# UCLALibrary/jp2-bucketeer

Measured on AMD Instinct MI355X. Metric: encoded megapixels/sec (node), lossless 5/3 + lossy 9/7, at 1/2/4/8 MI355X, higher is better.
Workload: dtype f32+i32

## Files before the change

jp2-bucketeer_amd/csrc/t1.hip:

```cpp
#include <hip/hip_runtime.h>

#include <algorithm>
#include <cstdlib>
#include <cstring>

#include "device_common.h"
#include "gpu_encoder.h"

namespace jp2hip {

enum { CX_RL = 17, CX_UNI = 18, CX_PAD = 19 };
constexpr uint8_t kPadDecision = CX_PAD << 1;



constexpr int kCmWaves = 2;

__device__ __forceinline__ int order_bucket(uint32_t n) {
    const uint32_t v = n + 1u;
    const int e = 31 - __clz(v);
    constexpr int kLog = kOrderSub == 16 ? 4 : 3;
    const int f = e >= kLog ? (int)((v >> (e - kLog)) & (kOrderSub - 1u)) : (int)((v << (kLog - e)) & (kOrderSub - 1u));
    return kOrderBuckets - 1 - min(kOrderBuckets - 1, kOrderSub * e + f);
}


constexpr uint64_t kStripeTop = 0x1111111111111111ull;
constexpr uint64_t kStripeBot = 0x8888888888888888ull;

__device__ __forceinline__ uint64_t col_left(uint64_t x, int) { return wave_shr1(x); }
__device__ __forceinline__ uint64_t col_right(uint64_t x, int) { return wave_shl1(x); }

struct Nbr8 {
    uint64_t UL, U, UR, L, R, DL, D, DR;
};
__device__ __forceinline__ Nbr8 nbr8(uint64_t Vb, uint64_t Va, uint64_t LVb, uint64_t RVb, uint64_t LVa,
                                     uint64_t RVa) {
    Nbr8 n;
    n.UL = LVb << 1;
    n.U = Vb << 1;
    n.UR = ((RVb << 1) & kStripeTop) | ((RVa << 1) & ~kStripeTop);
    n.L = LVb;
    n.R = RVa;
    n.DL = ((LVa >> 1) & kStripeBot) | ((LVb >> 1) & ~kStripeBot);
    n.D = Va >> 1;
    n.DR = RVa >> 1;
    return n;
}

template <uint32_t TT>
__device__ __forceinline__ uint64_t b3(uint64_t a, uint64_t b, uint64_t c) {
    const uint32_t lo = __builtin_amdgcn_bitop3_b32((uint32_t)a, (uint32_t)b, (uint32_t)c, TT);
    const uint32_t hi = __builtin_amdgcn_bitop3_b32((uint32_t)(a >> 32), (uint32_t)(b >> 32), (uint32_t)(c >> 32), TT);
    return ((uint64_t)hi << 32) | lo;
}

struct Ctx4 {
    uint64_t b0, b1, b2, b3;
};
__device__ __forceinline__ Ctx4 zc_masks(int band, const Nbr8 &n) {
    const uint64_t u = n.UL | n.UR, d = n.DL | n.DR, dge1 = u | d;
    const uint64_t s2a = n.DL & n.DR;
    const uint64_t dge2 = b3<0xEA>(u, d, b3<0xEA>(n.UL, n.UR, s2a));
    Ctx4 z;
    if (band == 3) {
        const uint64_t dge3 = b3<0xEA>(s2a, u, (n.UL & n.UR) & d);
        const uint64_t a = n.L | n.R, c = n.U | n.D, hvge1 = a | c;
        const uint64_t hvge2 = b3<0xEA>(a, c, b3<0xEA>(n.L, n.R, n.U & n.D));
        const uint64_t d2 = b3<0x30>(dge2, dge3, dge3), d1 = b3<0x30>(dge1, dge2, dge2);
        const uint64_t hv1 = b3<0x30>(hvge1, hvge2, hvge2);
        z.b3 = dge3;
        z.b2 = b3<0xEA>(d1, hvge1, d2);
        z.b1 = b3<0xAE>(dge1, hvge2, b3<0xBA>(d1, hvge1, d2));
        z.b0 = b3<0xEA>(d2, hvge1, b3<0x72>(d1, dge1, hv1));
    } else {
        const uint64_t A1 = band == 1 ? n.U : n.L, A2 = band == 1 ? n.D : n.R;
        const uint64_t B1 = band == 1 ? n.L : n.U, B2 = band == 1 ? n.R : n.D;
        const uint64_t e = b3<0x30>(dge1, dge2, dge2);
        const uint64_t x = A1 ^ A2;
        z.b3 = A1 & A2;
        z.b2 = b3<0x3E>(A1, A2, B1 & B2);
        z.b1 = b3<0xEA>(x, B1 | B2 | dge1, b3<0x02>(A1, A2, b3<0x3E>(B1, B2, dge2)));
        z.b0 = b3<0xEA>(x, b3<0xFD>(B1, B2, dge1), b3<0x02>(A1, A2, b3<0x3E>(B1, B2, e)));
    }
    return z;
}

struct Sc4 {
    uint64_t b0, b1, b2, xr;
};
__device__ __forceinline__ void sc_pair(uint64_t As, uint64_t An, uint64_t Bs, uint64_t Bn, uint64_t &p, uint64_t &n) {
    const uint64_t nA = As & An, nB = Bs & Bn;
    const uint64_t pA = b3<0x30>(As, An, An), pB = b3<0x30>(Bs, Bn, Bn);
    p = b3<0xBA>(pB, nA, b3<0x10>(As, An, nB));
    n = b3<0xBA>(nB, pA, b3<0x30>(nA, pB, pB));
}
__device__ __forceinline__ Sc4 sc_masks(uint64_t Ls, uint64_t Ln, uint64_t Rs, uint64_t Rn, uint64_t Us, uint64_t Un,
                                        uint64_t Ds, uint64_t Dn) {
    uint64_t hp, hn, vp, vn;
    sc_pair(Ls, Ln, Rs, Rn, hp, hn);
    sc_pair(Us, Un, Ds, Dn, vp, vn);
    const uint64_t hnz = hp | hn, vnz = vp | vn;
    const uint64_t opp = b3<0xEA>(hn, vp, hp & vn);
    Sc4 c;
    c.b0 = ~(hnz ^ vnz);
    c.b1 = b3<0xAE>(hnz, vnz, opp);
    c.b2 = b3<0x30>(hnz, opp, opp);
    c.xr = b3<0xF2>(hn, hnz, vn);
    return c;
}


constexpr int kRingBytes = 4096;
constexpr int kRingGuard = 4;
constexpr int kRingWords = kRingBytes / 4 + kRingGuard;
constexpr int kCm3Blocks = 4096;

__device__ __forceinline__ uint32_t spread4(uint32_t nib) { return (nib * 0x00204081u) & 0x01010101u; }
__device__ __forceinline__ uint32_t spread4s(uint32_t nib, int k) {
    return __umul24(nib << k, 0x00204081u) & (0x01010101u << k);
}
__device__ __forceinline__ uint32_t nibw(uint32_t w, int sh) { return __builtin_amdgcn_ubfe(w, (uint32_t)sh, 4u); }

struct Ring {
    uint32_t *r;
    uint8_t *out;
    int pos, fl;
};

template <int NW>
__device__ __forceinline__ void ring_or(const Ring &g, uint32_t at, uint32_t o0, uint32_t o1, uint32_t o2,
                                        uint32_t n) {
    const uint32_t t = at & 3u;
    const uint32_t sel = 0x07060504u - __builtin_amdgcn_perm(0u, t, 0u);
    uint32_t *q = g.r + ((at >> 2) & (uint32_t)(kRingBytes / 4 - 1));
    if (n) {
        atomicOr(q, o0 << (8u * t));
        atomicOr(q + 1, __builtin_amdgcn_perm(o1, o0, sel));
        if (NW >= 3) atomicOr(q + 2, __builtin_amdgcn_perm(o2, o1, sel));
        if (NW >= 4) atomicOr(q + 3, __builtin_amdgcn_perm(0u, o2, sel));
    }
}

template <int NW>
__device__ __forceinline__ void ring_put2(Ring &g, uint32_t a0, uint32_t a1, uint32_t a2, uint32_t na, uint32_t b0,
                                          uint32_t b1, uint32_t b2, uint32_t nb) {
    const uint32_t n = na | (nb << 16);
    int v = (int)n;
    v += __builtin_amdgcn_update_dpp(0, v, 0x111, 0xf, 0xf, false);
    v += __builtin_amdgcn_update_dpp(0, v, 0x112, 0xf, 0xf, false);
    v += __builtin_amdgcn_update_dpp(0, v, 0x114, 0xf, 0xf, false);
    v += __builtin_amdgcn_update_dpp(0, v, 0x118, 0xf, 0xf, false);
    v += __builtin_amdgcn_update_dpp(0, v, 0x142, 0xa, 0xf, false);
    v += __builtin_amdgcn_update_dpp(0, v, 0x143, 0xc, 0xf, false);
    const uint32_t tot = (uint32_t)__builtin_amdgcn_readlane(v, 63);
    const uint32_t ex = (uint32_t)v - n;
    const uint32_t ta = tot & 0xFFFFu;
    ring_or<NW>(g, (uint32_t)g.pos + (ex & 0xFFFFu), a0, a1, a2, na);
    ring_or<NW>(g, (uint32_t)g.pos + ta + (ex >> 16), b0, b1, b2, nb);
    g.pos += (int)(ta + (tot >> 16));
}

__device__ __forceinline__ void ring_drain(Ring &g, int upto, int lane) {
    if (lane < kRingGuard) {
        const uint32_t gv = g.r[kRingBytes / 4 + lane];
        if (gv) {
            g.r[lane] |= gv;
            g.r[kRingBytes / 4 + lane] = 0u;
        }
    }
    __builtin_amdgcn_wave_barrier();
    for (int o = g.fl + 16 * lane; o < upto; o += 1024) {
        uint4 *src = (uint4 *)((uint8_t *)g.r + (o & (kRingBytes - 1)));
        const uint4 v = *src;
        *src = make_uint4(0u, 0u, 0u, 0u);
        *(uint4 *)(g.out + o) = v;
    }
    g.fl = __builtin_amdgcn_readfirstlane(upto);
}

__device__ __forceinline__ void ring_step(Ring &g, int lane) {
    if (__builtin_amdgcn_readfirstlane(g.pos - g.fl) >= 1024) ring_drain(g, g.fl + 1024, lane);
}

__device__ __forceinline__ void ring_pass_end(Ring &g, int lane) {
    const int end = (g.pos + 15) & ~15;
    if (lane < end - g.pos) ((uint8_t *)g.r)[(g.pos + lane) & (kRingBytes - 1)] = kPadDecision;
    ring_drain(g, end, lane);
    g.pos = end;
}

struct Half {
    uint32_t mem, bb, z0, z1, z2, z3, c0, c1, c2, xs, x;
};
__device__ __forceinline__ Half half_of(int hf, uint64_t mem, uint64_t bb, const Ctx4 &z, const Sc4 &sc, uint64_t xs,
                                        uint64_t x) {
    const int sh = hf * 32;
    return Half{(uint32_t)(mem >> sh),  (uint32_t)(bb >> sh),    (uint32_t)(z.b0 >> sh), (uint32_t)(z.b1 >> sh),
                (uint32_t)(z.b2 >> sh), (uint32_t)(z.b3 >> sh),  (uint32_t)(sc.b0 >> sh), (uint32_t)(sc.b1 >> sh),
                (uint32_t)(sc.b2 >> sh), (uint32_t)(xs >> sh), (uint32_t)(x >> sh)};
}
__device__ __forceinline__ uint32_t spread_or(uint32_t w, int sh, int k, uint32_t acc) {
    const uint32_t nib = nibw(w, sh);
    if (k <= 2) return (__umul24(nib, 0x00204081u << k) & (0x01010101u << k)) | acc;
    return spread4s(nib, k) | acc;
}
__device__ __forceinline__ void zc_sg_bytes(const Half &m, int sh, uint32_t &zc, uint32_t &sg) {
    zc = spread_or(m.bb, sh, 0, 0u);
    zc = spread_or(m.z0, sh, 1, zc);
    zc = spread_or(m.z1, sh, 2, zc);
    zc = spread_or(m.z2, sh, 3, zc);
    zc = spread_or(m.z3, sh, 4, zc);
    sg = spread_or(m.xs, sh, 0, 0x10101010u);
    sg = spread_or(m.c0, sh, 1, sg);
    sg = spread_or(m.c1, sh, 2, sg);
    sg = spread_or(m.c2, sh, 3, sg);
}

__device__ __forceinline__ void spp_stripe(const Half &m, int sh, const uint2 *lut, uint32_t &o0, uint32_t &o1,
                                           uint32_t &n) {
    const uint32_t mem = nibw(m.mem, sh);
    uint32_t zc, sg;
    zc_sg_bytes(m, sh, zc, sg);
    const uint32_t K = mem | ((mem & nibw(m.bb, sh)) << 4);
    const uint2 sel = lut[K];
    o0 = __builtin_amdgcn_perm(sg, zc, sel.x);
    o1 = __builtin_amdgcn_perm(sg, zc, sel.y);
    n = (uint32_t)__popc(K);
}
__device__ __forceinline__ void mrp_stripe(uint32_t wm, uint32_t wb, uint32_t wf, uint32_t wa, int sh,
                                           const uint2 *lut, uint32_t &o0, uint32_t &n) {
    const uint32_t mem = nibw(wm, sh);
    const uint32_t f = spread4(nibw(wf, sh));
    const uint32_t mr = (0x20202020u - (f << 2)) | spread_or(wa, sh, 1, spread4(nibw(wb, sh)));
    o0 = __builtin_amdgcn_perm(0u, mr, lut[mem].x);
    n = (uint32_t)__popc(mem);
}
__device__ __forceinline__ void cup_stripe(const Half &m, int sh, const uint2 *lut, uint32_t &o0, uint32_t &o1,
                                           uint32_t &o2, uint32_t &n) {
    const uint32_t mem = nibw(m.mem, sh);
    uint32_t zc, sg;
    zc_sg_bytes(m, sh, zc, sg);
    const uint32_t bb = nibw(m.bb, sh);
    const bool rl = mem == 0xFu && nibw(m.x, sh) == 0u;
    const uint32_t r = __builtin_ctz(bb | 16u);
    const uint32_t mr = rl ? (0xEu << r) & 0xFu : mem;
    const uint32_t K = mr | ((mr & bb) << 4);
    const uint2 sel = lut[K];
    o0 = __builtin_amdgcn_perm(sg, zc, sel.x);
    o1 = __builtin_amdgcn_perm(sg, zc, sel.y);
    o2 = 0u;
    n = (uint32_t)__popc(K);
    if (rl) {
        if (bb == 0u) {
            o0 = (uint32_t)(CX_RL << 1);
            n = 1;
        } else {
            o2 = o1;
            o1 = o0;
            o0 = (uint32_t)((CX_RL << 1) | 1) | ((uint32_t)((CX_UNI << 1) | (r >> 1)) << 8) |
                 ((uint32_t)((CX_UNI << 1) | (r & 1u)) << 16) | (((sg >> (8 * r)) & 0xFFu) << 24);
            n += 4;
        }
    }
}

__device__ __forceinline__ uint32_t cm_plane(const T1CmArgs &a, Ring &g, const uint2 *lut, int lane, int b, int k,
                                             int p, int P, int w, int h, int band, const uint64_t *CT, uint64_t B,
                                             uint64_t S0, uint64_t S1, uint64_t S2, uint64_t SG, uint64_t LSG,
                                             uint64_t RSG) {
    const bool lossless = a.lossless != 0;
    const bool vl = lane < w;
    const uint64_t VR = vl ? (h >= 64 ? ~0ull : ((1ull << h) - 1ull)) : 0ull;
    const int nstripes = (h + 3) >> 2;
    g.out = a.stream + a.slot_off[b] + (size_t)k * plane_stream_cap(w, h);
    g.pos = 0;
    g.fl = 0;
    int n_spp = 0, n_mrp = 0;
    const bool spp = p < P - 1;
    const uint64_t LS1 = col_left(S1, lane), RS1 = col_right(S1, lane);
    uint64_t N = 0, memS = 0;
    if (spp) {
        for (;;) {
            const uint64_t Vb = S1 | N, LVb = col_left(Vb, lane), RVb = col_right(Vb, lane);
            const Nbr8 nb = nbr8(Vb, S1, LVb, RVb, LS1, RS1);
            const uint64_t cand = ~S1 & VR & (nb.UL | nb.U | nb.UR | nb.L | nb.R | nb.DL | nb.D | nb.DR);
            const uint64_t Nn = cand & B;
            if (!__any(Nn != N)) {
                memS = cand;
                break;
            }
            N = Nn;
        }
        {
            const uint64_t Vb = S1 | N, LVb = col_left(Vb, lane), RVb = col_right(Vb, lane);
            const Nbr8 nb = nbr8(Vb, S1, LVb, RVb, LS1, RS1);
            const Ctx4 z = zc_masks(band, nb);
            const Sc4 sc = sc_masks(nb.L, LSG, nb.R, RSG, nb.U, SG << 1, nb.D, SG >> 1);
            for (int hf = 0; hf * 8 < nstripes; hf++) {
                const Half m = half_of(hf, memS, B, z, sc, SG ^ sc.xr, 0);
                for (int s4 = 0; s4 < 8 && hf * 8 + s4 < nstripes; s4 += 2) {
                    const int sh = s4 * 4;
                    const bool hb = hf * 8 + s4 + 1 < nstripes;
                    if (!__any(nibw(m.mem, sh) | (hb ? nibw(m.mem, sh + 4) : 0u))) continue;
                    uint32_t a0, a1, ca, b0 = 0, b1 = 0, cb = 0;
                    spp_stripe(m, sh, lut, a0, a1, ca);
                    if (hb) spp_stripe(m, sh + 4, lut, b0, b1, cb);
                    ring_put2<3>(g, a0, a1, 0u, ca, b0, b1, 0u, cb);
                    ring_step(g, lane);
                }
            }
        }
        n_spp = g.pos;
        ring_pass_end(g, lane);
        const int mrp0 = g.pos;
        {
            const uint64_t Pst = S1 | N, LP = col_left(Pst, lane), RP = col_right(Pst, lane);
            const uint64_t anyn = (Pst << 1) | (Pst >> 1) | LP | RP | (LP << 1) | (RP << 1) | (LP >> 1) | (RP >> 1);
            const uint64_t memM = S1 & VR, fr = S1 & ~S2, fa = fr & anyn;
            for (int hf = 0; hf * 8 < nstripes; hf++) {
                const int hs = hf * 32;
                const uint32_t wm = (uint32_t)(memM >> hs), wb = (uint32_t)(B >> hs), wf = (uint32_t)(fr >> hs),
                               wa = (uint32_t)(fa >> hs);
                for (int s4 = 0; s4 < 8 && hf * 8 + s4 < nstripes; s4 += 2) {
                    const int sh = s4 * 4;
                    const bool hb = hf * 8 + s4 + 1 < nstripes;
                    if (!__any(nibw(wm, sh) | (hb ? nibw(wm, sh + 4) : 0u))) continue;
                    uint32_t a0, ca, b0 = 0, cb = 0;
                    mrp_stripe(wm, wb, wf, wa, sh, lut, a0, ca);
                    if (hb) mrp_stripe(wm, wb, wf, wa, sh + 4, lut, b0, cb);
                    ring_put2<2>(g, a0, 0u, 0u, ca, b0, 0u, 0u, cb);
                    ring_step(g, lane);
                }
            }
        }
        n_mrp = g.pos - mrp0;
        ring_pass_end(g, lane);
    }
    const int cup0 = g.pos;
    {
        const uint64_t Pst = S1 | N, LP = col_left(Pst, lane), RP = col_right(Pst, lane);
        const uint64_t LS0 = col_left(S0, lane), RS0 = col_right(S0, lane);
        const Nbr8 nb = nbr8(S0, Pst, LS0, RS0, LP, RP);
        const Ctx4 z = zc_masks(band, nb);
        const Sc4 sc = sc_masks(nb.L, LSG, nb.R, RSG, nb.U, SG << 1, nb.D, SG >> 1);
        const uint64_t memC = ~S1 & ~memS & VR;
        const uint64_t side = LS0 | RP, above = S0 | LS0 | RS0, below = Pst | LP | RP;
        const uint64_t blk = side | ((above << 1) & kStripeTop) | ((below >> 1) & kStripeBot);
        for (int hf = 0; hf * 8 < nstripes; hf++) {
            const Half m = half_of(hf, memC, B, z, sc, SG ^ sc.xr, blk);
            for (int s4 = 0; s4 < 8 && hf * 8 + s4 < nstripes; s4 += 2) {
                const int sh = s4 * 4;
                const bool hb = hf * 8 + s4 + 1 < nstripes;
                if (!__any(nibw(m.mem, sh) | (hb ? nibw(m.mem, sh + 4) : 0u))) continue;
                uint32_t a0, a1, a2, ca, b0 = 0, b1 = 0, b2 = 0, cb = 0;
                cup_stripe(m, sh, lut, a0, a1, a2, ca);
                if (hb) cup_stripe(m, sh + 4, lut, b0, b1, b2, cb);
                ring_put2<4>(g, a0, a1, a2, ca, b0, b1, b2, cb);
                ring_step(g, lane);
            }
        }
    }
    const int n_cup = g.pos - cup0;
    ring_pass_end(g, lane);
    int64_t dspp = 0;
    if (spp && __any(N != 0ull)) {
        const uint32_t nl = (uint32_t)__popcll(N);
        int64_t sv = (int64_t)nl << p;
#pragma unroll 4
        for (int q = 0; q < p; q++) sv += (int64_t)__popcll(N & CT[(size_t)q * 64 + lane]) << q;
        const int64_t nN = (int64_t)wave_sum_u32(nl);
        sv = wave_sum64(sv);
        dspp = (lossless && p == 0) ? 4 * nN
                                    : ((12 * sv + (6 * (lossless ? 0 : 1) - 9 * ((int64_t)1 << p)) * nN) << p);
    }
    if (lane == 0) {
        uint4 cnt;
        cnt.x = (uint32_t)n_spp;
        cnt.y = (uint32_t)n_mrp;
        cnt.z = (uint32_t)n_cup;
        cnt.w = 0;
        a.counts[(size_t)b * 32 + k] = cnt;
        a.dspp[(size_t)b * 32 + k] = dspp;
    }
    return (uint32_t)(n_spp + n_mrp + n_cup);
}

__device__ __forceinline__ uint2 cm_selectors(int K) {
    uint64_t sel = 0x0C0C0C0C0C0C0C0Cull;
    int n = 0;
#pragma unroll
    for (int q = 0; q < 8; q++) {
        const int bit = (q & 1) ? 4 + (q >> 1) : (q >> 1);
        if ((K >> bit) & 1) {
            sel = (sel & ~(0xFFull << (8 * n))) | ((uint64_t)((q & 1) ? 4 + (q >> 1) : (q >> 1)) << (8 * n));
            n++;
        }
    }
    return make_uint2((uint32_t)sel, (uint32_t)(sel >> 32));
}

struct CmBlk {
    int b, P, c, w, h, Mb, band;
    uint64_t bp_off, slot;
};
__device__ __forceinline__ CmBlk cm_blk_load(const T1CmArgs &a, int b) {
    const BlockDesc d = a.blocks[b];
    CmBlk k;
    k.b = b;
    k.P = a.P[b];
    k.c = (int)(a.acc[b] >> 40);
    k.w = d.w;
    k.h = d.h;
    k.Mb = d.Mb;
    k.band = d.band;
    k.bp_off = d.bp_off;
    k.slot = a.slot_off[b];
    return k;
}
struct CmMasks {
    uint64_t SG, B;
};
__device__ __forceinline__ CmMasks cm_masks_load(const T1CmArgs &a, const CmBlk &k, int lane) {
    const uint64_t *CT = a.bp + k.bp_off;
    CmMasks m;
    m.SG = CT[(size_t)k.Mb * 64 + lane];
    m.B = CT[(size_t)(k.P - 1) * 64 + lane];
    return m;
}

#ifdef JP2HIP_CM_WAVES_PER_EU
__global__ void __launch_bounds__(64 * kCmWaves) __attribute__((amdgpu_waves_per_eu(JP2HIP_CM_WAVES_PER_EU))) k_t1_cm3(T1CmArgs a) {
#else
__global__ void __launch_bounds__(64 * kCmWaves) k_t1_cm3(T1CmArgs a) {
#endif
    __shared__ uint2 lut[256];
    __shared__ uint32_t rings[kCmWaves][kRingWords];
    const int lane = threadIdx.x & 63;
    const int wv = __builtin_amdgcn_readfirstlane(threadIdx.x >> 6);
    for (int K = threadIdx.x; K < 256; K += 64 * kCmWaves) lut[K] = cm_selectors(K);
    for (int i = threadIdx.x; i < kCmWaves * kRingWords; i += 64 * kCmWaves) (&rings[0][0])[i] = 0u;
    __syncthreads();
    const int nblk = a.kmax > 0 ? (int)a.dfill[0] : 0;
    Ring g;
    g.r = rings[wv];
    const int stride = gridDim.x * kCmWaves;
    int bi = blockIdx.x * kCmWaves + wv;
    if (bi >= nblk) return;
    CmBlk cur = cm_blk_load(a, a.dlist[bi]);
    CmMasks mk = cm_masks_load(a, cur, lane);
    int idx_next = bi + stride < nblk ? a.dlist[bi + stride] : -1;
    for (;;) {
        const int b = cur.b, P = cur.P, c = cur.c, w = cur.w, h = cur.h, band = cur.band;
        const bool vl = lane < w;
        const uint64_t *CT = a.bp + cur.bp_off;
        uint64_t Bl = mk.B;
        const uint64_t SG = vl ? mk.SG : 0ull;
        const uint64_t LSG = col_left(SG, lane), RSG = col_right(SG, lane);
        uint64_t S1 = 0, S2 = 0;
        uint32_t tot = 0;
        const uint32_t cap = plane_stream_cap(w, h);
        uint8_t *out = a.stream + cur.slot;
        CmBlk nxt;
        int idx_after = -1;
        for (int k = 0; k < c; k++) {
            const int p = P - 1 - k;
            const uint64_t B = vl ? Bl : 0ull, S0 = S1 | B;
            if (k + 1 < c) Bl = CT[(size_t)(p - 1) * 64 + lane];
            if (k == 0 && idx_next >= 0) {
                nxt = cm_blk_load(a, idx_next);
                if (bi + 2 * stride < nblk) idx_after = a.dlist[bi + 2 * stride];
            }
            g.out = out + (size_t)k * cap;
            g.pos = 0;
            g.fl = 0;
            tot += cm_plane(a, g, lut, lane, b, k, p, P, w, h, band, CT, B, S0, S1, S2, SG, LSG, RSG);
#ifdef JP2HIP_BURN_VALU
            {
                uint32_t x = (uint32_t)B ^ (uint32_t)lane;
                for (int i = 0; i < JP2HIP_BURN_VALU; i++) x = (x ^ (uint32_t)i) + (x << 3);
                if (x == 0x9E3779B9u) a.counts[(size_t)b * 32 + k].w = x;
            }
#endif
#ifdef JP2HIP_BURN_SLEEP
            __builtin_amdgcn_s_sleep(JP2HIP_BURN_SLEEP);
#endif
            S2 = S1;
            S1 = S0;
        }
        const bool more = idx_next >= 0;
        if (more) mk = cm_masks_load(a, nxt, lane);
        if (lane == 0) {
            a.acc[b] = tot;
            const int bk = order_bucket(tot);
            a.bslots[(size_t)bk * a.nb + atomicAdd(&a.bfill[bk], 1u)] = b;
        }
        if (!more) break;
        bi += stride;
        cur = nxt;
        idx_next = idx_after;
    }
}

__constant__ uint16_t c_qe[47] = {
    0x5601, 0x3401, 0x1801, 0x0AC1, 0x0521, 0x0221, 0x5601, 0x5401, 0x4801, 0x3801, 0x3001, 0x2401,
    0x1C01, 0x1601, 0x5601, 0x5401, 0x5101, 0x4801, 0x3801, 0x3401, 0x3001, 0x2801, 0x2401, 0x2201,
    0x1C01, 0x1801, 0x1601, 0x1401, 0x1201, 0x1101, 0x0AC1, 0x09C1, 0x08A1, 0x0521, 0x0441, 0x02A1,
    0x0221, 0x0141, 0x0111, 0x0085, 0x0049, 0x0025, 0x0015, 0x0009, 0x0005, 0x0001, 0x5601};
__constant__ uint8_t c_nmps[47] = {1,  2,  3,  4,  5,  38, 7,  8,  9,  10, 11, 12, 13, 29, 15, 16,
                                   17, 18, 19, 20, 21, 22, 23, 24, 25, 26, 27, 28, 29, 30, 31, 32,
                                   33, 34, 35, 36, 37, 38, 39, 40, 41, 42, 43, 44, 45, 45, 46};
__constant__ uint8_t c_nlps[47] = {1,  6,  9,  12, 29, 33, 6,  14, 14, 14, 17, 18, 20, 21, 14, 14,
                                   15, 16, 17, 18, 19, 19, 20, 21, 22, 23, 24, 25, 26, 27, 28, 29,
                                   30, 31, 32, 33, 34, 35, 36, 37, 38, 39, 40, 41, 42, 43, 46};

struct Mq {
    uint32_t C, A, B;
    int CT, bp, cap;
    uint8_t *out;
};

__device__ __forceinline__ void mq_byteout(Mq &m) {
    uint32_t B = m.B;
    if (B != 0xFF && m.C >= 0x8000000u) {
        B++;
        m.C &= 0x7FFFFFFu;
    }
    if (m.bp >= 0 && m.bp < m.cap) m.out[m.bp] = (uint8_t)B;
    m.bp++;
    if (B == 0xFF) {
        m.B = m.C >> 20;
        m.C &= 0xFFFFFu;
        m.CT = 7;
    } else {
        m.B = m.C >> 19;
        m.C &= 0x7FFFFu;
        m.CT = 8;
    }
}

__device__ __forceinline__ uint32_t ring_at(int bp, uint32_t lb) {
    uint32_t r;
    asm("v_bfi_b32 %0, 63, %1, %2" : "=v"(r) : "v"(bp), "v"(lb));
    return r;
}

__device__ __forceinline__ void ring_byteout(Mq &m, uint8_t *ring, uint32_t lb) {
    uint32_t B = m.B;
    if (B != 0xFF && m.C >= 0x8000000u) {
        B++;
        m.C &= 0x7FFFFFFu;
    }
    ring[ring_at(m.bp, lb)] = (uint8_t)B;
    m.bp++;
    const bool ff = B == 0xFF;
    m.B = ff ? (m.C >> 20) : (m.C >> 19);
    m.C &= ff ? 0xFFFFFu : 0x7FFFFu;
    m.CT = ff ? 7 : 8;
}

constexpr int kMqChunk = 16;
#ifndef JP2HIP_MQ_EXP
#define JP2HIP_MQ_EXP 0
#endif
constexpr uint32_t kPadWord = 0x01010101u * kPadDecision;
constexpr int kQeShift = 16;
#ifndef JP2HIP_MQ_SCHED
#define JP2HIP_MQ_SCHED 1
#endif
#ifndef JP2HIP_MQ_PASS_PREFETCH
#define JP2HIP_MQ_PASS_PREFETCH 1
#endif


__device__ __forceinline__ uint32_t mq_word(int e) {
    return ((uint32_t)c_qe[e >> 1] << kQeShift) | ((uint32_t)e << 3) | (uint32_t)(e & 1);
}

__device__ __forceinline__ uint32_t mq_model(uint32_t &A, const uint32_t t, const uint8_t *tab, const uint32_t d,
                                             uint32_t *code) {
#if JP2HIP_MQ_EXP == 3
    const uint2 nx = make_uint2(t ^ 0x10008u, t ^ 0x20010u);
#else
    const uint2 nx = *(const uint2 *)(tab + (t & 0x3F8u));
#endif
    const uint32_t qe = t & 0xFFFF0000u;
    const bool isM = d == (t & 1u);
    const uint32_t A1 = A - qe;
    const bool keep = isM != (A1 < qe);
    const uint32_t An = keep ? A1 : qe;
    const bool ren = !isM || A1 < 0x80000000u;
    const uint32_t n = (uint32_t)__builtin_clz(An);
    A = An << n;
    const uint32_t cw = (keep ? qe : 0u) | n;
#if JP2HIP_MQ_SCHED
    __builtin_amdgcn_sched_barrier(0);
#endif
    *code = cw;
    return ren ? (isM ? nx.x : nx.y) : t;
}

template <bool TWO>
__device__ __forceinline__ void mq_code(Mq &m, const uint32_t code, uint8_t *ring, uint32_t lb) {
    const uint32_t add = code >> kQeShift;
    const int n = (int)(code & 0x1Fu);
    const uint32_t C0 = m.C + add;
    const int CT = m.CT;
    const bool bo = n >= CT;
    const int s1 = min(n, CT);
    const uint32_t C1 = C0 << s1;
    const bool carry = (m.B != 0xFFu) && (C1 >= 0x8000000u);
    const uint32_t Bc = m.B + (carry ? 1u : 0u);
    const uint32_t C2 = carry ? (C1 & 0x7FFFFFFu) : C1;
    const bool ff = Bc == 0xFFu;
    const uint32_t sh = ff ? 20u : 19u;
    ring[ring_at(m.bp, lb)] = (uint8_t)Bc;
    uint32_t Cx = bo ? (C2 & ((1u << sh) - 1u)) : C1;
    int CTx = bo ? 27 - (int)sh : CT - n;
    int rem = n - s1;
    m.B = bo ? (C2 >> sh) : m.B;
    m.bp += bo ? 1 : 0;
    if (TWO && bo && rem >= CTx) {
        m.C = Cx << CTx;
        rem -= CTx;
        ring_byteout(m, ring, lb);
        Cx = m.C;
        CTx = m.CT;
    }
    m.C = Cx << rem;
    m.CT = CTx - rem;
}

__device__ __forceinline__ void ring_flush(const Mq &m, const uint8_t *ring, uint32_t lb, int off, int &fl) {
    while (m.bp - fl >= 16) {
        uint4 v;
        v.x = *(const uint32_t *)(ring + ring_at(fl, lb));
        v.y = *(const uint32_t *)(ring + ring_at(fl + 4, lb));
        v.z = *(const uint32_t *)(ring + ring_at(fl + 8, lb));
        v.w = *(const uint32_t *)(ring + ring_at(fl + 12, lb));
        if (fl - off + 16 <= m.cap) *(uint4 *)(m.out + (fl - off)) = v;
        fl += 16;
    }
}

__device__ __forceinline__ int mq_flush(Mq &m) {
    uint32_t tempc = m.C + m.A;
    m.C |= 0xFFFFu;
    if (m.C >= tempc) m.C -= 0x8000u;
    m.C <<= m.CT;
    mq_byteout(m);
    m.C <<= m.CT;
    mq_byteout(m);
    if (m.B != 0xFF) {
        if (m.bp >= 0 && m.bp < m.cap) m.out[m.bp] = (uint8_t)m.B;
        m.bp++;
    }
    return m.bp;
}

struct MqShared {
    uint2 mqt[94];
    uint32_t cxs[20 * 64];
    uint32_t rings[64 * 16];
    union {
        uint32_t bbase[kOrderBuckets + 1];
        uint32_t code[2][kMqChunk][64];
    };
    int32_t segs[2][64];
    uint32_t finA[64];
    int32_t blk[64];
    int32_t more[2];
#ifdef JP2HIP_MQ_LDS_PAD
    uint8_t pad_[JP2HIP_MQ_LDS_PAD];
#endif
};

__device__ __forceinline__ void mq_modeller(const T1MqArgs &a, MqShared &sh) {
    const int lane = threadIdx.x & 63;
    const int b = sh.blk[lane];
    uint32_t *cx = sh.cxs + lane;
    const uint8_t *mqt = (const uint8_t *)sh.mqt;
    const uint32_t w0 = mq_word(0);
#pragma unroll
    for (int q = 0; q < 19; q++) cx[q * 64] = w0;
    cx[CX_PAD * 64] = 0u;
    cx[0] = mq_word(2 * 4);
    cx[CX_RL * 64] = mq_word(2 * 3);
    cx[CX_UNI * 64] = mq_word(2 * 46);
    uint32_t A = 0x8000u << kQeShift;
    int nseg = 0, s = 0, k = 0, pass = 2, left = 0, Pt = 0;
    uint32_t cap = 0;
    const uint8_t *sbase = nullptr;
    const uint4 *cntp = nullptr, *ptr = nullptr;
    const int64_t *dspp = nullptr, *dref = nullptr, *dsig = nullptr;
    int64_t *D = nullptr;
    const uint4 pad4 = make_uint4(kPadWord, kPadWord, kPadWord, kPadWord);
    uint4 cnt = make_uint4(0u, 0u, 0u, 0u), cur = pad4, nx1 = pad4;
    int64_t ndec = 0;
#if JP2HIP_MQ_PASS_PREFETCH
    int pf_pass = 0, pf_k = 0, pf_valid = 0;
    uint4 pf_cnt = cnt, pf_cur = pad4, pf_nx1 = pad4;
    const uint4 *pf_ptr = nullptr;
    auto prefetch = [&]() {
        pf_valid = 0;
        if (s + 1 >= nseg) return;
        const int np = pass == 2 ? 0 : pass + 1, nk = pass == 2 ? k + 1 : k;
        const uint4 nc = np == 0 ? cntp[nk] : cnt;
        const int o_mrp = ((int)cnt.x + 15) & ~15;
        const int o_cup = (o_mrp + (int)cnt.y + 15) & ~15;
        pf_ptr = (const uint4 *)(sbase + (size_t)nk * cap + (np == 0 ? 0 : (np == 1 ? o_mrp : o_cup)));
        pf_cur = pf_ptr[0];
        pf_nx1 = pf_ptr[1];
        pf_pass = np;
        pf_k = nk;
        pf_cnt = nc;
        pf_valid = 1;
    };
#endif
    if (b >= 0) {
        const BlockDesc d = a.blocks[b];
        Pt = a.P[b];
        const int P = Pt - a.pmin[b];
        nseg = 3 * P - 2;
        D = a.dists + (size_t)b * kMaxPasses;
        cap = plane_stream_cap(d.w, d.h);
        sbase = a.stream + a.slot_off[b];
        cntp = a.counts + (size_t)b * 32;
        dspp = a.dspp + (size_t)b * 32;
        dref = a.dref + (size_t)b * 32;
        dsig = a.dsig + (size_t)b * 32;
        cnt = cntp[0];
        ptr = (const uint4 *)sbase;
        left = (int)cnt.z;
        ndec = left;
        cur = ptr[0];
        if (left > 16) nx1 = ptr[1];
#if JP2HIP_MQ_PASS_PREFETCH
        prefetch();
#endif
    }
    uint64_t cyc_wait = 0;
    const uint64_t cyc0 = __builtin_readcyclecounter();
    for (int it = 0;; it++) {
        while (left <= 0 && s < nseg) {
#if JP2HIP_MQ_PASS_PREFETCH
            if (++s >= nseg) break;
            pass = pf_pass;
            k = pf_k;
            cnt = pf_cnt;
            ptr = pf_ptr;
            cur = pf_cur;
            nx1 = pf_nx1;
            left = pass == 0 ? (int)cnt.x : (pass == 1 ? (int)cnt.y : (int)cnt.z);
            ndec += left;
            prefetch();
#else
            const int p = Pt - 1 - k;
            D[s] = pass == 0 ? dspp[k] : (pass == 1 ? dref[p] : dsig[p] - dspp[k]);
            if (++s >= nseg) break;
            pass = pass == 2 ? 0 : pass + 1;
            if (pass == 0) {
                k++;
                cnt = cntp[k];
            }
            const int o_mrp = ((int)cnt.x + 15) & ~15;
            const int o_cup = (o_mrp + (int)cnt.y + 15) & ~15;
            ptr = (const uint4 *)(sbase + (size_t)k * cap + (pass == 0 ? 0 : (pass == 1 ? o_mrp : o_cup)));
            left = pass == 0 ? (int)cnt.x : (pass == 1 ? (int)cnt.y : (int)cnt.z);
            ndec += left;
            cur = ptr[0];
            nx1 = left > 16 ? ptr[1] : pad4;
#endif
        }
        const bool active = s < nseg;
        const int buf = it & 1;
        sh.segs[buf][lane] = s;
        if (!__any(active)) {
            sh.finA[lane] = A >> kQeShift;
            if (lane == 0) sh.more[buf] = 0;
// ... 194 lines not shown
```

Measured before the change: 34670.

## Fuse SPP, MRP and cleanup passes into one stripe sweep with per-pass rings

The three coding passes (significance propagation, magnitude refinement, cleanup) per bit-plane used to run as three separate stripe sweeps through one shared LDS ring. Now a single sweep emits all three into separate per-pass LDS rings. The MRP/SPP output offsets are precomputed from wave-wide popcounts, and the cleanup neighbourhood is built by selecting the SPP neighbourhood under the SPP membership mask. This removes two of the three sweeps and the repeated mask and context setup, but it raises register pressure and LDS use and adds extra scans per stripe. The default waves-per-EU attribute is also now always set to 4.

```diff
diff --git a/jp2-bucketeer_amd/csrc/t1.hip b/jp2-bucketeer_amd/csrc/t1.hip
--- a/jp2-bucketeer_amd/csrc/t1.hip
+++ b/jp2-bucketeer_amd/csrc/t1.hip
@@ -111,9 +111,13 @@
 }
 
 
-constexpr int kRingBytes = 4096;
 constexpr int kRingGuard = 4;
-constexpr int kRingWords = kRingBytes / 4 + kRingGuard;
+constexpr int kRingSpp = 2048, kDrainSpp = 1024, kStripeSpp = 512;
+constexpr int kRingMrp = 1024, kDrainMrp = 512, kStripeMrp = 256;
+constexpr int kRingCup = 2048, kDrainCup = 512, kStripeCup = 768;
+constexpr int kRingWordsSpp = kRingSpp / 4 + kRingGuard, kRingWordsMrp = kRingMrp / 4 + kRingGuard,
+              kRingWordsCup = kRingCup / 4 + kRingGuard;
+constexpr int kWaveRingWords = kRingWordsSpp + kRingWordsMrp + kRingWordsCup;
 constexpr int kCm3Blocks = 4096;
 
 __device__ __forceinline__ uint32_t spread4(uint32_t nib) { return (nib * 0x00204081u) & 0x01010101u; }
@@ -122,18 +126,18 @@
 }
 __device__ __forceinline__ uint32_t nibw(uint32_t w, int sh) { return __builtin_amdgcn_ubfe(w, (uint32_t)sh, 4u); }
 
+template <int BYTES>
 struct Ring {
     uint32_t *r;
-    uint8_t *out;
     int pos, fl;
 };
 
-template <int NW>
-__device__ __forceinline__ void ring_or(const Ring &g, uint32_t at, uint32_t o0, uint32_t o1, uint32_t o2,
+template <int NW, int BYTES>
+__device__ __forceinline__ void ring_or(const Ring<BYTES> &g, uint32_t at, uint32_t o0, uint32_t o1, uint32_t o2,
                                         uint32_t n) {
     const uint32_t t = at & 3u;
     const uint32_t sel = 0x07060504u - __builtin_amdgcn_perm(0u, t, 0u);
-    uint32_t *q = g.r + ((at >> 2) & (uint32_t)(kRingBytes / 4 - 1));
+    uint32_t *q = g.r + ((at >> 2) & (uint32_t)(BYTES / 4 - 1));
     if (n) {
         atomicOr(q, o0 << (8u * t));
         atomicOr(q + 1, __builtin_amdgcn_perm(o1, o0, sel));
@@ -142,64 +146,44 @@
     }
 }
 
-template <int NW>
-__device__ __forceinline__ void ring_put2(Ring &g, uint32_t a0, uint32_t a1, uint32_t a2, uint32_t na, uint32_t b0,
-                                          uint32_t b1, uint32_t b2, uint32_t nb) {
-    const uint32_t n = na | (nb << 16);
-    int v = (int)n;
-    v += __builtin_amdgcn_update_dpp(0, v, 0x111, 0xf, 0xf, false);
-    v += __builtin_amdgcn_update_dpp(0, v, 0x112, 0xf, 0xf, false);
-    v += __builtin_amdgcn_update_dpp(0, v, 0x114, 0xf, 0xf, false);
-    v += __builtin_amdgcn_update_dpp(0, v, 0x118, 0xf, 0xf, false);
-    v += __builtin_amdgcn_update_dpp(0, v, 0x142, 0xa, 0xf, false);
-    v += __builtin_amdgcn_update_dpp(0, v, 0x143, 0xc, 0xf, false);
-    const uint32_t tot = (uint32_t)__builtin_amdgcn_readlane(v, 63);
-    const uint32_t ex = (uint32_t)v - n;
-    const uint32_t ta = tot & 0xFFFFu;
-    ring_or<NW>(g, (uint32_t)g.pos + (ex & 0xFFFFu), a0, a1, a2, na);
-    ring_or<NW>(g, (uint32_t)g.pos + ta + (ex >> 16), b0, b1, b2, nb);
-    g.pos += (int)(ta + (tot >> 16));
-}
-
-__device__ __forceinline__ void ring_drain(Ring &g, int upto, int lane) {
+template <int BYTES>
+__device__ __forceinline__ void ring_drain(Ring<BYTES> &g, uint8_t *out, int upto, int lane) {
     if (lane < kRingGuard) {
-        const uint32_t gv = g.r[kRingBytes / 4 + lane];
+        const uint32_t gv = g.r[BYTES / 4 + lane];
         if (gv) {
             g.r[lane] |= gv;
-            g.r[kRingBytes / 4 + lane] = 0u;
+            g.r[BYTES / 4 + lane] = 0u;
         }
     }
     __builtin_amdgcn_wave_barrier();
     for (int o = g.fl + 16 * lane; o < upto; o += 1024) {
-        uint4 *src = (uint4 *)((uint8_t *)g.r + (o & (kRingBytes - 1)));
+        uint4 *src = (uint4 *)((uint8_t *)g.r + (o & (BYTES - 1)));
         const uint4 v = *src;
         *src = make_uint4(0u, 0u, 0u, 0u);
-        *(uint4 *)(g.out + o) = v;
+        *(uint4 *)(out + o) = v;
     }
     g.fl = __builtin_amdgcn_readfirstlane(upto);
 }
 
-__device__ __forceinline__ void ring_step(Ring &g, int lane) {
-    if (__builtin_amdgcn_readfirstlane(g.pos - g.fl) >= 1024) ring_drain(g, g.fl + 1024, lane);
-}
-
-__device__ __forceinline__ void ring_pass_end(Ring &g, int lane) {
+template <int DRAIN, int ADD, int BYTES>
+__device__ __forceinline__ void ring_step(Ring<BYTES> &g, uint8_t *out, int lane) {
+    static_assert(DRAIN % 16 == 0 && DRAIN - 1 + ADD < BYTES, "ring_step: pending bytes must fit the ring");
+    const int pend = __builtin_amdgcn_readfirstlane(g.pos - g.fl);
+    if (pend >= DRAIN) ring_drain(g, out, g.fl + (pend & ~15), lane);
+}
+
+template <int BYTES>
+__device__ __forceinline__ void ring_pass_end(Ring<BYTES> &g, uint8_t *out, int lane) {
     const int end = (g.pos + 15) & ~15;
-    if (lane < end - g.pos) ((uint8_t *)g.r)[(g.pos + lane) & (kRingBytes - 1)] = kPadDecision;
-    ring_drain(g, end, lane);
+    if (end == g.fl) return;
+    if (lane < end - g.pos) ((uint8_t *)g.r)[(g.pos + lane) & (BYTES - 1)] = kPadDecision;
+    ring_drain(g, out, end, lane);
     g.pos = end;
 }
 
 struct Half {
-    uint32_t mem, bb, z0, z1, z2, z3, c0, c1, c2, xs, x;
-};
-__device__ __forceinline__ Half half_of(int hf, uint64_t mem, uint64_t bb, const Ctx4 &z, const Sc4 &sc, uint64_t xs,
-                                        uint64_t x) {
-    const int sh = hf * 32;
-    return Half{(uint32_t)(mem >> sh),  (uint32_t)(bb >> sh),    (uint32_t)(z.b0 >> sh), (uint32_t)(z.b1 >> sh),
-                (uint32_t)(z.b2 >> sh), (uint32_t)(z.b3 >> sh),  (uint32_t)(sc.b0 >> sh), (uint32_t)(sc.b1 >> sh),
-                (uint32_t)(sc.b2 >> sh), (uint32_t)(xs >> sh), (uint32_t)(x >> sh)};
-}
+    uint32_t ms, mm, mc, bb, z0, z1, z2, z3, c0, c1, c2, xs, x, fr, fa;
+};
 __device__ __forceinline__ uint32_t spread_or(uint32_t w, int sh, int k, uint32_t acc) {
     const uint32_t nib = nibw(w, sh);
     if (k <= 2) return (__umul24(nib, 0x00204081u << k) & (0x01010101u << k)) | acc;
@@ -217,74 +201,171 @@
     sg = spread_or(m.c2, sh, 3, sg);
 }
 
-__device__ __forceinline__ void spp_stripe(const Half &m, int sh, const uint2 *lut, uint32_t &o0, uint32_t &o1,
-                                           uint32_t &n) {
-    const uint32_t mem = nibw(m.mem, sh);
-    uint32_t zc, sg;
-    zc_sg_bytes(m, sh, zc, sg);
-    const uint32_t K = mem | ((mem & nibw(m.bb, sh)) << 4);
-    const uint2 sel = lut[K];
-    o0 = __builtin_amdgcn_perm(sg, zc, sel.x);
-    o1 = __builtin_amdgcn_perm(sg, zc, sel.y);
-    n = (uint32_t)__popc(K);
-}
-__device__ __forceinline__ void mrp_stripe(uint32_t wm, uint32_t wb, uint32_t wf, uint32_t wa, int sh,
-                                           const uint2 *lut, uint32_t &o0, uint32_t &n) {
-    const uint32_t mem = nibw(wm, sh);
-    const uint32_t f = spread4(nibw(wf, sh));
-    const uint32_t mr = (0x20202020u - (f << 2)) | spread_or(wa, sh, 1, spread4(nibw(wb, sh)));
-    o0 = __builtin_amdgcn_perm(0u, mr, lut[mem].x);
-    n = (uint32_t)__popc(mem);
-}
-__device__ __forceinline__ void cup_stripe(const Half &m, int sh, const uint2 *lut, uint32_t &o0, uint32_t &o1,
-                                           uint32_t &o2, uint32_t &n) {
-    const uint32_t mem = nibw(m.mem, sh);
-    uint32_t zc, sg;
-    zc_sg_bytes(m, sh, zc, sg);
-    const uint32_t bb = nibw(m.bb, sh);
-    const bool rl = mem == 0xFu && nibw(m.x, sh) == 0u;
+__device__ __forceinline__ uint32_t mrp_bytes(const Half &m, uint32_t mem, int sh, const uint2 *lut) {
+    const uint32_t f = spread4(nibw(m.fr, sh));
+    const uint32_t mr = (0x20202020u - (f << 2)) | spread_or(m.fa, sh, 1, spread4(nibw(m.bb, sh)));
+    return __builtin_amdgcn_perm(0u, mr, lut[mem].x);
+}
+__device__ __forceinline__ bool cup_rl(uint32_t mem, uint32_t x) { return mem == 0xFu && x == 0u; }
+__device__ __forceinline__ void cup_count(uint32_t mem, uint32_t bb, uint32_t x, uint32_t &K, uint32_t &n) {
+    const bool rl = cup_rl(mem, x);
     const uint32_t r = __builtin_ctz(bb | 16u);
     const uint32_t mr = rl ? (0xEu << r) & 0xFu : mem;
-    const uint32_t K = mr | ((mr & bb) << 4);
+    K = mr | ((mr & bb) << 4);
+    n = (uint32_t)__popc(K) + (rl ? (bb ? 4u : 1u) : 0u);
+}
+__device__ __forceinline__ void cup_bytes(uint32_t mem, uint32_t bb, uint32_t x, uint32_t K, uint32_t zc, uint32_t sg,
+                                          const uint2 *lut, uint32_t &o0, uint32_t &o1, uint32_t &o2) {
     const uint2 sel = lut[K];
     o0 = __builtin_amdgcn_perm(sg, zc, sel.x);
     o1 = __builtin_amdgcn_perm(sg, zc, sel.y);
     o2 = 0u;
-    n = (uint32_t)__popc(K);
-    if (rl) {
+    if (cup_rl(mem, x)) {
         if (bb == 0u) {
             o0 = (uint32_t)(CX_RL << 1);
-            n = 1;
         } else {
+            const uint32_t r = __builtin_ctz(bb);
             o2 = o1;
             o1 = o0;
             o0 = (uint32_t)((CX_RL << 1) | 1) | ((uint32_t)((CX_UNI << 1) | (r >> 1)) << 8) |
                  ((uint32_t)((CX_UNI << 1) | (r & 1u)) << 16) | (((sg >> (8 * r)) & 0xFFu) << 24);
-            n += 4;
-        }
-    }
-}
-
-__device__ __forceinline__ uint32_t cm_plane(const T1CmArgs &a, Ring &g, const uint2 *lut, int lane, int b, int k,
-                                             int p, int P, int w, int h, int band, const uint64_t *CT, uint64_t B,
-                                             uint64_t S0, uint64_t S1, uint64_t S2, uint64_t SG, uint64_t LSG,
-                                             uint64_t RSG) {
+        }
+    }
+}
+
+__device__ __forceinline__ Nbr8 nbr_select(uint64_t sel, const Nbr8 &x, const Nbr8 &y) {
+    Nbr8 n;
+    n.UL = b3<0xCA>(sel, x.UL, y.UL);
+    n.U = b3<0xCA>(sel, x.U, y.U);
+    n.UR = b3<0xCA>(sel, x.UR, y.UR);
+    n.L = b3<0xCA>(sel, x.L, y.L);
+    n.R = b3<0xCA>(sel, x.R, y.R);
+    n.DL = b3<0xCA>(sel, x.DL, y.DL);
+    n.D = b3<0xCA>(sel, x.D, y.D);
+    n.DR = b3<0xCA>(sel, x.DR, y.DR);
+    return n;
+}
+
+struct PassRings {
+    Ring<kRingSpp> S;
+    Ring<kRingMrp> M;
+    Ring<kRingCup> C;
+};
+struct SweepMasks {
+    uint64_t memS, memM, memC, B, xs, blk, fr, fa;
+    Ctx4 z;
+    Sc4 sc;
+};
+
+struct StripeCnt {
+    uint32_t ms, mm, mc, bb, x, Ks, Kc, nc, n;
+};
+template <bool SPP>
+__device__ __forceinline__ StripeCnt stripe_counts(const Half &m, int sh, bool aC) {
+    StripeCnt c;
+    c.ms = SPP ? nibw(m.ms, sh) : 0u;
+    c.mm = SPP ? nibw(m.mm, sh) : 0u;
+    c.mc = nibw(m.mc, sh);
+    c.bb = nibw(m.bb, sh);
+    c.x = nibw(m.x, sh);
+    c.Ks = c.ms | ((c.ms & c.bb) << 4);
+    c.Kc = 0;
+    c.nc = 0;
+    if (aC) cup_count(c.mc, c.bb, c.x, c.Kc, c.nc);
+    c.n = SPP ? (uint32_t)__popc(c.Ks) | ((uint32_t)__popc(c.mm) << 10) | (c.nc << 20) : c.nc;
+    return c;
+}
+template <bool SPP>
+__device__ __forceinline__ void cm_sweep(PassRings &g, const SweepMasks &k, uint8_t *out, const uint2 *lut, int lane,
+                                         int nstripes) {
+    for (int hf = 0; hf * 8 < nstripes; hf++) {
+        const int hs = hf * 32;
+        const Half m{(uint32_t)(k.memS >> hs),  (uint32_t)(k.memM >> hs),  (uint32_t)(k.memC >> hs),
+                     (uint32_t)(k.B >> hs),     (uint32_t)(k.z.b0 >> hs),  (uint32_t)(k.z.b1 >> hs),
+                     (uint32_t)(k.z.b2 >> hs),  (uint32_t)(k.z.b3 >> hs),  (uint32_t)(k.sc.b0 >> hs),
+                     (uint32_t)(k.sc.b1 >> hs), (uint32_t)(k.sc.b2 >> hs), (uint32_t)(k.xs >> hs),
+                     (uint32_t)(k.blk >> hs),   (uint32_t)(k.fr >> hs),    (uint32_t)(k.fa >> hs)};
+        for (int s4 = 0; s4 < 8 && hf * 8 + s4 < nstripes; s4 += 2) {
+            const int sh = s4 * 4;
+            const bool aS = SPP && __any(__builtin_amdgcn_ubfe(m.ms, (uint32_t)sh, 8u));
+            const bool aM = SPP && __any(__builtin_amdgcn_ubfe(m.mm, (uint32_t)sh, 8u));
+            const bool aC = __any(__builtin_amdgcn_ubfe(m.mc, (uint32_t)sh, 8u));
+            if (!(aS || aM || aC)) continue;
+            const StripeCnt A = stripe_counts<SPP>(m, sh, aC), B = stripe_counts<SPP>(m, sh + 4, aC);
+            uint32_t exA, exB, totA, totB;
+            if (SPP) {
+                const uint32_t vA = wave_incl_scan(A.n), vB = wave_incl_scan(B.n);
+                totA = (uint32_t)__builtin_amdgcn_readlane((int)vA, 63);
+                totB = (uint32_t)__builtin_amdgcn_readlane((int)vB, 63);
+                exA = vA - A.n;
+                exB = vB - B.n;
+            } else {
+                const uint32_t n = A.n | (B.n << 16), v = wave_incl_scan(n);
+                const uint32_t tot = (uint32_t)__builtin_amdgcn_readlane((int)v, 63), ex = v - n;
+                totA = tot & 0xFFFFu;
+                totB = tot >> 16;
+                exA = ex & 0xFFFFu;
+                exB = ex >> 16;
+            }
+            if (aS || aC) {
+                uint32_t zcA, sgA, zcB, sgB;
+                zc_sg_bytes(m, sh, zcA, sgA);
+                zc_sg_bytes(m, sh + 4, zcB, sgB);
+                if (aS) {
+                    const uint2 selA = lut[A.Ks], selB = lut[B.Ks];
+                    const uint32_t tA = totA & 0x3FFu;
+                    ring_or<3>(g.S, (uint32_t)g.S.pos + (exA & 0x3FFu), __builtin_amdgcn_perm(sgA, zcA, selA.x),
+                               __builtin_amdgcn_perm(sgA, zcA, selA.y), 0u, A.Ks);
+                    ring_or<3>(g.S, (uint32_t)g.S.pos + tA + (exB & 0x3FFu), __builtin_amdgcn_perm(sgB, zcB, selB.x),
+                               __builtin_amdgcn_perm(sgB, zcB, selB.y), 0u, B.Ks);
+                    g.S.pos += (int)(tA + (totB & 0x3FFu));
+                    ring_step<kDrainSpp, 2 * kStripeSpp>(g.S, out, lane);
+                }
+                if (aC) {
+                    uint32_t a0, a1, a2, b0, b1, b2;
+                    cup_bytes(A.mc, A.bb, A.x, A.Kc, zcA, sgA, lut, a0, a1, a2);
+                    cup_bytes(B.mc, B.bb, B.x, B.Kc, zcB, sgB, lut, b0, b1, b2);
+                    const uint32_t tA = SPP ? totA >> 20 : totA;
+                    ring_or<4>(g.C, (uint32_t)g.C.pos + (SPP ? exA >> 20 : exA), a0, a1, a2, A.nc);
+                    ring_or<4>(g.C, (uint32_t)g.C.pos + tA + (SPP ? exB >> 20 : exB), b0, b1, b2, B.nc);
+                    g.C.pos += (int)(tA + (SPP ? totB >> 20 : totB));
+                    ring_step<kDrainCup, 2 * kStripeCup>(g.C, out, lane);
+                }
+            }
+            if (aM) {
+                const uint32_t tA = (totA >> 10) & 0x3FFu;
+                ring_or<2>(g.M, (uint32_t)g.M.pos + ((exA >> 10) & 0x3FFu), mrp_bytes(m, A.mm, sh, lut), 0u, 0u, A.mm);
+                ring_or<2>(g.M, (uint32_t)g.M.pos + tA + ((exB >> 10) & 0x3FFu), mrp_bytes(m, B.mm, sh + 4, lut), 0u,
+                           0u, B.mm);
+                g.M.pos += (int)(tA + ((totB >> 10) & 0x3FFu));
+                ring_step<kDrainMrp, 2 * kStripeMrp>(g.M, out, lane);
+            }
+        }
+    }
+}
+
+__device__ __forceinline__ uint32_t cm_plane(const T1CmArgs &a, uint32_t *ring, const uint2 *lut, int lane, int b,
+                                             int k, int p, int P, int w, int h, int band, const uint64_t *CT,
+                                             uint64_t B, uint64_t S0, uint64_t S1, uint64_t S2, uint64_t SG,
+                                             uint64_t LSG, uint64_t RSG) {
     const bool lossless = a.lossless != 0;
     const bool vl = lane < w;
     const uint64_t VR = vl ? (h >= 64 ? ~0ull : ((1ull << h) - 1ull)) : 0ull;
     const int nstripes = (h + 3) >> 2;
-    g.out = a.stream + a.slot_off[b] + (size_t)k * plane_stream_cap(w, h);
-    g.pos = 0;
-    g.fl = 0;
+    uint8_t *out = a.stream + a.slot_off[b] + (size_t)k * plane_stream_cap(w, h);
+    const bool spp = p < P - 1;
+    uint64_t N = 0, memS = 0, LP = 0, RP = 0;
     int n_spp = 0, n_mrp = 0;
-    const bool spp = p < P - 1;
-    const uint64_t LS1 = col_left(S1, lane), RS1 = col_right(S1, lane);
-    uint64_t N = 0, memS = 0;
+    Nbr8 nbS;
     if (spp) {
+        const uint64_t LS1 = col_left(S1, lane), RS1 = col_right(S1, lane);
         for (;;) {
-            const uint64_t Vb = S1 | N, LVb = col_left(Vb, lane), RVb = col_right(Vb, lane);
-            const Nbr8 nb = nbr8(Vb, S1, LVb, RVb, LS1, RS1);
-            const uint64_t cand = ~S1 & VR & (nb.UL | nb.U | nb.UR | nb.L | nb.R | nb.DL | nb.D | nb.DR);
+            const uint64_t Vb = S1 | N;
+            LP = col_left(Vb, lane);
+            RP = col_right(Vb, lane);
+            nbS = nbr8(Vb, S1, LP, RP, LS1, RS1);
+            const uint64_t cand =
+                ~S1 & VR & (nbS.UL | nbS.U | nbS.UR | nbS.L | nbS.R | nbS.DL | nbS.D | nbS.DR);
             const uint64_t Nn = cand & B;
             if (!__any(Nn != N)) {
                 memS = cand;
@@ -292,77 +373,42 @@
             }
             N = Nn;
         }
-        {
-            const uint64_t Vb = S1 | N, LVb = col_left(Vb, lane), RVb = col_right(Vb, lane);
-            const Nbr8 nb = nbr8(Vb, S1, LVb, RVb, LS1, RS1);
-            const Ctx4 z = zc_masks(band, nb);
-            const Sc4 sc = sc_masks(nb.L, LSG, nb.R, RSG, nb.U, SG << 1, nb.D, SG >> 1);
-            for (int hf = 0; hf * 8 < nstripes; hf++) {
-                const Half m = half_of(hf, memS, B, z, sc, SG ^ sc.xr, 0);
-                for (int s4 = 0; s4 < 8 && hf * 8 + s4 < nstripes; s4 += 2) {
-                    const int sh = s4 * 4;
-                    const bool hb = hf * 8 + s4 + 1 < nstripes;
-                    if (!__any(nibw(m.mem, sh) | (hb ? nibw(m.mem, sh + 4) : 0u))) continue;
-                    uint32_t a0, a1, ca, b0 = 0, b1 = 0, cb = 0;
-                    spp_stripe(m, sh, lut, a0, a1, ca);
-                    if (hb) spp_stripe(m, sh + 4, lut, b0, b1, cb);
-                    ring_put2<3>(g, a0, a1, 0u, ca, b0, b1, 0u, cb);
-                    ring_step(g, lane);
-                }
-            }
-        }
-        n_spp = g.pos;
-        ring_pass_end(g, lane);
-        const int mrp0 = g.pos;
-        {
-            const uint64_t Pst = S1 | N, LP = col_left(Pst, lane), RP = col_right(Pst, lane);
-            const uint64_t anyn = (Pst << 1) | (Pst >> 1) | LP | RP | (LP << 1) | (RP << 1) | (LP >> 1) | (RP >> 1);
-            const uint64_t memM = S1 & VR, fr = S1 & ~S2, fa = fr & anyn;
-            for (int hf = 0; hf * 8 < nstripes; hf++) {
-                const int hs = hf * 32;
-                const uint32_t wm = (uint32_t)(memM >> hs), wb = (uint32_t)(B >> hs), wf = (uint32_t)(fr >> hs),
-                               wa = (uint32_t)(fa >> hs);
-                for (int s4 = 0; s4 < 8 && hf * 8 + s4 < nstripes; s4 += 2) {
-                    const int sh = s4 * 4;
-                    const bool hb = hf * 8 + s4 + 1 < nstripes;
-                    if (!__any(nibw(wm, sh) | (hb ? nibw(wm, sh + 4) : 0u))) continue;
-                    uint32_t a0, ca, b0 = 0, cb = 0;
-                    mrp_stripe(wm, wb, wf, wa, sh, lut, a0, ca);
-                    if (hb) mrp_stripe(wm, wb, wf, wa, sh + 4, lut, b0, cb);
-                    ring_put2<2>(g, a0, 0u, 0u, ca, b0, 0u, 0u, cb);
-                    ring_step(g, lane);
-                }
-            }
-        }
-        n_mrp = g.pos - mrp0;
-        ring_pass_end(g, lane);
-    }
-    const int cup0 = g.pos;
+        const uint32_t pk = wave_sum_u32((uint32_t)(__popcll(memS) + __popcll(memS & B)) |
+                                         ((uint32_t)__popcll(S1 & VR) << 16));
+        n_spp = (int)(pk & 0xFFFFu);
+        n_mrp = (int)(pk >> 16);
+    }
+    const uint64_t Pst = S1 | N;
+    const int o_mrp = (n_spp + 15) & ~15, o_cup = (o_mrp + n_mrp + 15) & ~15;
+    PassRings g{{ring, 0, 0}, {ring + kRingWordsSpp, o_mrp, o_mrp}, {ring + kRingWordsSpp + kRingWordsMrp, o_cup, o_cup}};
     {
-        const uint64_t Pst = S1 | N, LP = col_left(Pst, lane), RP = col_right(Pst, lane);
         const uint64_t LS0 = col_left(S0, lane), RS0 = col_right(S0, lane);
-        const Nbr8 nb = nbr8(S0, Pst, LS0, RS0, LP, RP);
+        Nbr8 nb = nbr8(S0, Pst, LS0, RS0, LP, RP);
+        if (spp) nb = nbr_select(memS, nbS, nb);
         const Ctx4 z = zc_masks(band, nb);
         const Sc4 sc = sc_masks(nb.L, LSG, nb.R, RSG, nb.U, SG << 1, nb.D, SG >> 1);
-        const uint64_t memC = ~S1 & ~memS & VR;
+        SweepMasks m;
+        m.memS = memS;
+        m.memM = S1 & VR;
+        m.memC = ~S1 & ~memS & VR;
+        m.B = B;
+        m.z = z;
+        m.sc = sc;
+        m.xs = SG ^ sc.xr;
         const uint64_t side = LS0 | RP, above = S0 | LS0 | RS0, below = Pst | LP | RP;
-        const uint64_t blk = side | ((above << 1) & kStripeTop) | ((below >> 1) & kStripeBot);
-        for (int hf = 0; hf * 8 < nstripes; hf++) {
-            const Half m = half_of(hf, memC, B, z, sc, SG ^ sc.xr, blk);
-            for (int s4 = 0; s4 < 8 && hf * 8 + s4 < nstripes; s4 += 2) {
-                const int sh = s4 * 4;
-                const bool hb = hf * 8 + s4 + 1 < nstripes;
-                if (!__any(nibw(m.mem, sh) | (hb ? nibw(m.mem, sh + 4) : 0u))) continue;
-                uint32_t a0, a1, a2, ca, b0 = 0, b1 = 0, b2 = 0, cb = 0;
-                cup_stripe(m, sh, lut, a0, a1, a2, ca);
-                if (hb) cup_stripe(m, sh + 4, lut, b0, b1, b2, cb);
-                ring_put2<4>(g, a0, a1, a2, ca, b0, b1, b2, cb);
-                ring_step(g, lane);
-            }
-        }
-    }
-    const int n_cup = g.pos - cup0;
-    ring_pass_end(g, lane);
+        m.blk = side | ((above << 1) & kStripeTop) | ((below >> 1) & kStripeBot);
+        const uint64_t anyn = (Pst << 1) | (Pst >> 1) | LP | RP | (LP << 1) | (RP << 1) | (LP >> 1) | (RP >> 1);
+        m.fr = S1 & ~S2;
+        m.fa = m.fr & anyn;
+        if (spp)
+            cm_sweep<true>(g, m, out, lut, lane, nstripes);
+        else
+            cm_sweep<false>(g, m, out, lut, lane, nstripes);
+    }
+    const int n_cup = g.C.pos - o_cup;
+    ring_pass_end(g.S, out, lane);
+    ring_pass_end(g.M, out, lane);
+    ring_pass_end(g.C, out, lane);
     int64_t dspp = 0;
     if (spp && __any(N != 0ull)) {
         const uint32_t nl = (uint32_t)__popcll(N);
@@ -429,21 +475,19 @@
     return m;
 }
 
-#ifdef JP2HIP_CM_WAVES_PER_EU
+#ifndef JP2HIP_CM_WAVES_PER_EU
+#define JP2HIP_CM_WAVES_PER_EU 4
+#endif
 __global__ void __launch_bounds__(64 * kCmWaves) __attribute__((amdgpu_waves_per_eu(JP2HIP_CM_WAVES_PER_EU))) k_t1_cm3(T1CmArgs a) {
-#else
-__global__ void __launch_bounds__(64 * kCmWaves) k_t1_cm3(T1CmArgs a) {
-#endif
     __shared__ uint2 lut[256];
-    __shared__ uint32_t rings[kCmWaves][kRingWords];
+    __shared__ uint32_t rings[kCmWaves][kWaveRingWords];
     const int lane = threadIdx.x & 63;
     const int wv = __builtin_amdgcn_readfirstlane(threadIdx.x >> 6);
     for (int K = threadIdx.x; K < 256; K += 64 * kCmWaves) lut[K] = cm_selectors(K);
-    for (int i = threadIdx.x; i < kCmWaves * kRingWords; i += 64 * kCmWaves) (&rings[0][0])[i] = 0u;
+    for (int i = threadIdx.x; i < kCmWaves * kWaveRingWords; i += 64 * kCmWaves) (&rings[0][0])[i] = 0u;
     __syncthreads();
     const int nblk = a.kmax > 0 ? (int)a.dfill[0] : 0;
-    Ring g;
-    g.r = rings[wv];
+    uint32_t *ring = rings[wv];
     const int stride = gridDim.x * kCmWaves;
     int bi = blockIdx.x * kCmWaves + wv;
     if (bi >= nblk) return;
@@ -459,8 +503,6 @@
         const uint64_t LSG = col_left(SG, lane), RSG = col_right(SG, lane);
         uint64_t S1 = 0, S2 = 0;
         uint32_t tot = 0;
-        const uint32_t cap = plane_stream_cap(w, h);
-        uint8_t *out = a.stream + cur.slot;
         CmBlk nxt;
         int idx_after = -1;
         for (int k = 0; k < c; k++) {
@@ -471,10 +513,7 @@
                 nxt = cm_blk_load(a, idx_next);
                 if (bi + 2 * stride < nblk) idx_after = a.dlist[bi + 2 * stride];
             }
-            g.out = out + (size_t)k * cap;
-            g.pos = 0;
-            g.fl = 0;
-            tot += cm_plane(a, g, lut, lane, b, k, p, P, w, h, band, CT, B, S0, S1, S2, SG, LSG, RSG);
+            tot += cm_plane(a, ring, lut, lane, b, k, p, P, w, h, band, CT, B, S0, S1, S2, SG, LSG, RSG);
 #ifdef JP2HIP_BURN_VALU
             {
                 uint32_t x = (uint32_t)B ^ (uint32_t)lane;
```

Result: no change. 34400 (-0.8%).
